# facebookresearch/gtn

Hardware: AMD Instinct MI355X
Metric: CTC forward+backward losses/sec (T=1000, C=256) (higher is better)
Workload: dtype f32; 1 GPU; BASELINE config C3: compose(ctc_target, emissions)+forwardScore CTC loss fwd+bwd, T=1000, C=256, U=100, batch=512 per GPU; global_batch=512, parallelism=dp1 (utterance sharding, all_gather of losses), rccl_ranks=0

## Files before the change

gtn_amd/_capi.py:

```python
import ctypes as C
import os

c_graph = C.c_void_p
c_graph_p = C.POINTER(C.c_void_p)
c_i32_p = C.POINTER(C.c_int)
c_i64_p = C.POINTER(C.c_int64)
c_u8_p = C.POINTER(C.c_uint8)
c_f32_p = C.POINTER(C.c_float)

GRAD_FN = C.CFUNCTYPE(C.c_int, C.c_void_p, c_graph_p, C.c_int, c_graph)
CTX_FREE = C.CFUNCTYPE(None, C.c_void_p)

OK, INVALID_ARGUMENT, LOGIC_ERROR, RUNTIME_ERROR, OUT_OF_RANGE, DEVICE_ERROR = range(6)

_SIGS = {
    "gtnx_set_device": [C.c_int],
    "gtnx_get_device": [c_i32_p],
    "gtnx_set_stream": [C.c_void_p],
    "gtnx_compose_mode": [C.c_int, C.POINTER(C.c_int)],
    "gtnx_synchronize": [],
    "gtnx_memory_stats": [C.POINTER(C.c_uint64), C.POINTER(C.c_uint64)],
    "gtnx_empty_cache": [],
    "gtnx_reclaim": [],
    "gtnx_graph_create": [C.c_int, c_graph_p],
# ... 55 lines not shown
    "gtnx_compose": [c_graph, c_graph, c_graph_p],
    "gtnx_intersect": [c_graph, c_graph, c_graph_p],
    "gtnx_forward_score": [c_graph, c_graph_p],
    "gtnx_viterbi_score": [c_graph, c_graph_p],
    "gtnx_viterbi_path": [c_graph, c_graph_p],
    "gtnx_negate_n": [c_graph_p, C.c_int, c_graph_p],
    "gtnx_add_n": [c_graph_p, C.c_int, c_graph_p, C.c_int, c_graph_p],
    "gtnx_subtract_n": [c_graph_p, C.c_int, c_graph_p, C.c_int, c_graph_p],
    "gtnx_compose_n": [c_graph_p, C.c_int, c_graph_p, C.c_int, c_graph_p],
    "gtnx_intersect_n": [c_graph_p, C.c_int, c_graph_p, C.c_int, c_graph_p],
    "gtnx_forward_score_n": [c_graph_p, C.c_int, c_graph_p],
    "gtnx_viterbi_score_n": [c_graph_p, C.c_int, c_graph_p],
    "gtnx_viterbi_path_n": [c_graph_p, C.c_int, c_graph_p],
    "gtnx_items_n": [c_graph_p, C.c_int, C.c_void_p],
    "gtnx_items_device_n": [c_graph_p, C.c_int, C.c_void_p],
    "gtnx_grads_device_n": [c_graph_p, C.c_int, C.c_void_p, C.c_void_p],
    "gtnx_grads_bind_device_n": [c_graph_p, C.c_int, C.c_void_p, C.c_void_p],
    "gtnx_clone": [c_graph, C.c_int, c_graph_p],
    "gtnx_concat": [c_graph_p, C.c_int, c_graph_p],
    "gtnx_closure": [c_graph, c_graph_p],
    "gtnx_union": [c_graph_p, C.c_int, c_graph_p],
    "gtnx_batch_from_graphs": [c_graph_p, C.c_int, c_graph_p],
    "gtnx_batch_ctc_targets": [C.c_void_p, C.c_void_p, C.c_int, C.c_int, C.c_int, c_graph_p],
    "gtnx_batch_asg_force_align": [C.c_void_p, C.c_void_p, C.c_int, c_graph, C.c_int, c_graph_p],
    "gtnx_batch_linear": [C.c_int, C.c_int, C.c_int, C.c_int, C.c_void_p, C.c_int, c_graph_p],
    "gtnx_batch_linear_rows": [C.c_int, C.c_int, C.c_int, C.c_void_p, C.c_int, C.c_void_p, C.c_int, c_graph_p],
    "gtnx_batch_destroy": [c_graph],
    "gtnx_batch_size": [c_graph, c_i32_p],
    "gtnx_batch_get": [c_graph, C.c_int, c_graph_p],
    "gtnx_batch_negate": [c_graph, c_graph_p],
    "gtnx_batch_add": [c_graph, c_graph, c_graph_p],
    "gtnx_batch_subtract": [c_graph, c_graph, c_graph_p],
    "gtnx_batch_subtract_into": [c_graph, c_graph, C.c_void_p, c_graph_p],
    "gtnx_batch_compose": [c_graph, c_graph, c_graph_p],
    "gtnx_batch_intersect": [c_graph, c_graph, c_graph_p],
    "gtnx_batch_forward_score": [c_graph, c_graph_p],
    "gtnx_batch_viterbi_score": [c_graph, c_graph_p],
    "gtnx_batch_viterbi_path": [c_graph, c_graph_p],
    "gtnx_batch_viterbi_align": [c_graph, C.c_void_p, C.c_void_p, C.c_int64, C.c_void_p, C.c_void_p],
    "gtnx_batch_align_stats": [c_i64_p, c_i64_p],
    "gtnx_batch_viterbi_decode": [c_graph, c_graph, C.c_void_p, C.c_void_p, C.c_int64, C.c_void_p, C.c_void_p,
                                  C.c_void_p],
    "gtnx_batch_decode_stats": [c_i64_p, c_i64_p],
    "gtnx_batch_full_connect_stats": [c_i64_p, c_i64_p],
    "gtnx_batch_linear_decode": [c_graph, C.c_void_p, C.c_int, C.c_void_p, C.c_int64, C.c_void_p, C.c_void_p,
                                 C.c_void_p, C.c_void_p],
# ... 85 lines not shown
```

gtn_amd/criteria/criteria_capi.cpp:

```cpp
#include <cstring>
#include <string>

#include <map>
#include <mutex>

#include "asg_criterion.h"
#include "ctc_criterion.h"
#include "edit_distance.h"

#define GTN_EXPORT extern "C" __attribute__((visibility("default")))

namespace {
thread_local std::string g_err;

template <class F>
int guarded(F&& body) {
  try {
    body();
    return 0;
  } catch (const std::exception& e) {
    g_err = e.what();
    return -1;
  }
}
// ... 78 lines not shown
                                    const void* weights, void* grad) {
  return guarded([&] {
    if (!weights || !grad) throw std::invalid_argument("gtn_ctc_score_grad_n: null weights or grad");
    gtn::criteria::ctcScoreBatch(emissions, B, T, C, blank, frames, tokens, lengths, N, L, max_length, nullptr, weights,
                                 grad);
  });
}

GTN_EXPORT int gtn_edit_distance_n(const void* hyp, const void* hyp_lengths, const void* ref, const void* ref_lengths,
                                   int B, int N, int L, int U, void* dist, void* ops) {
  return guarded([&] { gtn::criteria::editDistanceBatch(hyp, hyp_lengths, ref, ref_lengths, B, N, L, U, dist, ops); });
}

GTN_EXPORT int gtn_ctc_loss_target_grads_n(const void* emissions, const int* targets, const int* lengths, int B, int T,
                                           int C, int blank, void* loss, void* grad, void* target_grad,
                                           const int64_t* target_grad_offsets) {
  return guarded([&] {
    gtn::Batch ctcs;
    gtn::criteria::ctcLossBatch(emissions, targets, lengths, B, T, C, blank, loss, grad, true, nullptr, &ctcs);
    if (target_grad) ctcs.gradsToDevice(target_grad, target_grad_offsets);
  });
}

namespace {
void asg_loss_impl(const void* emissions, const int* targets, const int* lengths, int B, int T, int N, const void* trans_w,
                   const int* frames, void* loss, void* grad_em, void* grad_trans) {
  if (frames)
    for (int b = 0; b < B; ++b)
      if (frames[b] < 1 || frames[b] > T) throw std::invalid_argument("[gtn_asg_loss_frames_n] a frame count outside 1 .. T");
  std::lock_guard<std::mutex> lk(g_loss_transitions.mu);
  gtn::Graph& trans = transitions_for(g_loss_transitions, N, grad_trans != nullptr);
  trans.setCalcGrad(grad_trans != nullptr);
  trans.zeroGrad();
  trans.setWeightsDevice(trans_w);
  gtn::criteria::asgLossBatch(emissions, targets, lengths, B, T, N, trans, loss, grad_em, frames);
  if (grad_trans) {
    gtnx_graph_t h = trans.handle();
    int64_t off = 0;
    gtn::detail::check(gtnx_grads_device_n(&h, 1, grad_trans, &off));
  }
}
}

GTN_EXPORT int gtn_asg_loss_n(const void* emissions, const int* targets, const int* lengths, int B, int T, int N,
                              const void* trans_w, void* loss, void* grad_em, void* grad_trans) {
  return guarded([&] { asg_loss_impl(emissions, targets, lengths, B, T, N, trans_w, nullptr, loss, grad_em, grad_trans); });
// ... 31 lines not shown
```

gtn_amd/criteria/ctc_criterion.h:

```cpp
#pragma once

#include <chrono>
#include <cstdint>
#include <stdexcept>
#include <vector>

#include "gtn/gtn.h"

namespace gtn {
namespace criteria {

inline Graph ctcTargetGraph(const std::vector<int>& target, int blank = 0, bool calcGrad = true) {
  const int L = 2 * (int)target.size() + 1;
  std::vector<uint8_t> st(L, 0), ac(L, 0);
  std::vector<int> src, dst, lab;
  src.reserve(3 * L);
  dst.reserve(3 * L);
  lab.reserve(3 * L);
  for (int l = 0; l < L; l++) {
    const int idx = (l - 1) / 2;
    st[l] = l == 0;
    ac[l] = l == L - 1 || l + 2 == L;
    const int label = l % 2 ? target[idx] : blank;
    src.push_back(l), dst.push_back(l), lab.push_back(label);
// ... 10 lines not shown
struct CtcStepTimes {
  double build = 0, linear = 0, intersect = 0, forward = 0, backward = 0;
};

inline void ctcLossBatch(
    const void* emissions,
    const int* labels,
    const int* lengths,
    int B,
    int T,
    int C,
    int blank,
    void* lossDev,
    void* gradDev,
    bool targetGrad = true,
    CtcStepTimes* times = nullptr,
    Batch* targetsOut = nullptr,
    const int* frames = nullptr) {
  auto now = [] { return std::chrono::steady_clock::now(); };
  auto ms = [](auto a, auto b) { return std::chrono::duration<double, std::milli>(b - a).count(); };
  if (frames)
    for (int b = 0; b < B; ++b)
      if (frames[b] < 1 || frames[b] > T) throw std::invalid_argument("[ctcLossBatch] a frame count outside 1 .. T");
  auto t0 = now();
  Batch ctcs = Batch::ctcTargets(labels, lengths, B, blank, targetGrad);
  auto t1 = now();
  Batch ems = Batch::linear(B, T, C, emissions, gradDev != nullptr, true, frames);
  std::vector<int64_t> off(B);
  for (int b = 0; b < B; ++b) off[b] = (int64_t)b * T * C;
  if (gradDev) ems.bindGrads(gradDev, off.data());
  auto t2 = now();
  Batch comp = batched::intersect(ctcs, ems);
  auto t3 = now();
  Batch score = batched::forwardScore(comp);
  Batch norm = batched::forwardScore(ems);
  Batch losses = batched::subtract(norm, score, lossDev);
  auto t4 = now();
  if (gradDev) batched::backward(losses);
  auto t5 = now();
  if (times) *times = {ms(t0, t1), ms(t1, t2), ms(t2, t3), ms(t3, t4), ms(t4, t5)};
  losses.itemsToDevice(lossDev);
  if (gradDev) ems.gradsToDevice(gradDev, off.data());
  if (targetsOut) *targetsOut = std::move(ctcs);
}

inline void ctcLossBatch(
// ... 128 lines not shown
```

gtn_amd/csrc/band.hip:

```cpp
#include <hip/hip_runtime.h>

#include <algorithm>
#include <cstdlib>
#include <stdexcept>
#include <type_traits>

#include "kernels.h"

#ifdef GTNX_BAND_TIMING
__device__ long long g_band_timing[256];
#endif

namespace gtnx {
namespace {

constexpr float NEGF = -1.0e30f;
constexpr float DEADF = -1.0e29f;
constexpr float LOG2E = 1.44269504088896340736f;
constexpr double LN2 = 0.693147180559945309417;
constexpr int BW = 256;
constexpr int WG = 512;
constexpr int WGB = 768;
constexpr int NBE = 5;
constexpr int NBG = 7;
// ... 302 lines not shown

__device__ __forceinline__ float wave_max_of(const float* v, int n) {
  float mx = v[0];
  for (int j = 1; j < n; ++j) mx = fmaxf(mx, v[j]);
  return wave_max(mx);
}

template <int NPL, bool UNIT, int K, bool VEC>
__global__ __launch_bounds__(WG) void band_forward_kernel(const BandPair* __restrict__ pairs, int NSmax) {
#define GTNX_BAND_PAIR pairs[blockIdx.x]
#include "band_forward_body.inc"
#undef GTNX_BAND_PAIR
}
template <int NPL, bool UNIT, int K, bool VEC>
__global__ __launch_bounds__(WG) void band_forward_one_kernel(BandPair one, int NSmax) {
#define GTNX_BAND_PAIR one
#include "band_forward_body.inc"
#undef GTNX_BAND_PAIR
}

__device__ __forceinline__ BandPair band_patched(BandPair P, const BandPatch& pt) {
  if (pt.on) {
    const int b = P.bidx;
    P.delta = pt.delta + b;
    P.delta_norm = pt.delta_norm ? pt.delta_norm + b : nullptr;
    P.rowlse = pt.rowlse ? pt.rowlse + int64_t(b) * pt.M : nullptr;
    P.norm = nullptr;
    P.em_copy = nullptr;
    P.grad_em = pt.grad_em ? pt.grad_em + int64_t(b) * pt.A : nullptr;
    P.grad_fixed = pt.grad_fixed ? pt.grad_fixed + P.goff : nullptr;
  }
  return P;
}
template <int NPL, bool UNIT, bool GRADG, int K, bool VEC, bool BIG>
__global__ __launch_bounds__(WGB, BIG ? 3 : 6) void band_backward_kernel(const BandPair* __restrict__ pairs, int NSmax, BandPatch patch) {
#define GTNX_BAND_PAIR band_patched(pairs[blockIdx.x], patch)
#include "band_backward_body.inc"
#undef GTNX_BAND_PAIR
}
template <int NPL, bool UNIT, bool GRADG, int K, bool VEC, bool BIG>
__global__ __launch_bounds__(WGB, BIG ? 3 : 6) void band_backward_one_kernel(BandPair one, int NSmax) {
#define GTNX_BAND_PAIR one
#include "band_backward_body.inc"
#undef GTNX_BAND_PAIR
}


__global__ __launch_bounds__(512) void ctc_targets_kernel(const CtcTargetArgs* __restrict__ args, int blank) {
  const CtcTargetArgs a = args[blockIdx.x];
  __shared__ __attribute__((aligned(16))) int tl[256 + 4];
  __shared__ __attribute__((aligned(16))) int tk[256 + 4];
  const int N = a.N, U = (N - 1) >> 1, m = threadIdx.x;
  if (m < 260) {
    const int v = m < U ? a.labels[m] : 0x7fffffff;
    tl[m] = v;
    tk[m] = (m > 0 && m < U && v != a.labels[m - 1]) ? 1 : 0;
  }
  __syncthreads();
  if (m >= N) return;
  const bool odd = (m & 1) != 0;
  const int my = odd ? tl[(m - 1) >> 1] : blank;
  const int skip = odd ? tk[(m - 1) >> 1] : 0;
  const int mi = (m - 1) >> 1;
  const int before = odd ? mi : (m >> 1);
  int rank = 0, skips = 0;
  for (int o = 0; o < U; o += 4) {
    const gtnx_i4 l4 = *reinterpret_cast<const gtnx_i4*>(tl + o), k4 = *reinterpret_cast<const gtnx_i4*>(tk + o);
    const int lo[4] = {l4.x, l4.y, l4.z, l4.w}, ko[4] = {k4.x, k4.y, k4.z, k4.w};
#pragma unroll
    for (int k = 0; k < 4; ++k) {
      const bool front = o + k < before;
      rank += (lo[k] < my || (lo[k] == my && front)) ? 1 : 0;
      skips += front ? ko[k] : 0;
    }
  }
  rank += blank < my ? U + 1 : (blank == my ? (m + 1) >> 1 : 0);
  const int base = (m > 0 ? 2 * m - 1 : 0) + skips;
  GTNX_G BandNode* nd = const_cast<GTNX_G BandNode*>(a.nodes);
  nd[m].lab = my;
  nd[m].aid[0] = base;
  nd[m].aid[1] = m > 0 ? base + 1 : -1;
  nd[m].aid[2] = skip ? base + 2 : -1;
  a.nflags[m] = uint8_t((m == 0 ? NF_START : 0) | (m + 2 >= N ? NF_ACCEPT : 0));
  a.snode[rank] = m;
  a.slab[rank] = my;
  if (m == N - 1 && a.n_arcs) a.n_arcs[0] = base + 1 + (m > 0 ? 1 : 0) + skip;
}

__global__ __launch_bounds__(512) void band_viterbi_kernel(const BandDecode* __restrict__ pairs) {
  const BandDecode P = pairs[blockIdx.x];
  const int T = P.T, C = P.C, N = P.N, NS = P.NS;
  extern __shared__ float lds[];
  const float NINF = -__builtin_inff();
  float* a0 = lds;
  float* a1 = lds + 516;
  float* stage = lds + 1032;
  const int m = threadIdx.x;
  const GTNX_G gtnx_i4* nodes = reinterpret_cast<const GTNX_G gtnx_i4*>(P.nodes);
  int lab = 0;
  float wi[3] = {NINF, NINF, NINF};
  bool accept = false, start = false;
  if (m < N) {
    const gtnx_i4 q = nodes[m];
    lab = q.x >= 0 ? q.x : 0;
    const int a[3] = {q.y, q.z, q.w};
#pragma unroll
    for (int k = 0; k < 3; ++k)
      if (a[k] >= 0) wi[k] = P.w ? P.w[a[k]] : 0.0f;
    const uint8_t f = P.nflags[m];
// ... 539 lines not shown
    else if (max_nodes <= 128) launch_viterbi_wave<2>(d_pairs, n, ranked, st);
    else if (max_nodes <= 256) launch_viterbi_wave<4>(d_pairs, n, ranked, st);
    else launch_viterbi_wave<8>(d_pairs, n, ranked, st);
    return;
  }
  if (ranked) return;
  static std::atomic<uint64_t> done{0};
  if (gtnx_first_on_device first{done}) big_lds(band_viterbi_kernel);
  hipLaunchKernelGGL(band_viterbi_kernel, dim3(n), dim3(512), 4 * size_t(1032 + stage_floats) + 64, st, d_pairs);
}

void launch_asg_fal_targets(const AsgFalArgs* d_args, int n, int n_labels, hipStream_t st) {
  if (n > 0) hipLaunchKernelGGL(asg_fal_targets_kernel, dim3(n), dim3(512), 0, st, d_args, n_labels);
}
void launch_asg_fal_scatter(const float* g, const int* maps, const int64_t* tab, int n_seq, int64_t longest, float* trans_grad,
                            hipStream_t st) {
  if (n_seq > 0 && longest > 0)
    hipLaunchKernelGGL(asg_fal_scatter_kernel, dim3(unsigned(std::min<int64_t>((longest + 255) / 256, 64)), unsigned(n_seq)),
                       dim3(256), 0, st, g, maps, tab, trans_grad);
}
void launch_ctc_targets(const CtcTargetArgs* d_args, int n, int blank, hipStream_t st) {
  if (n > 0) hipLaunchKernelGGL(ctc_targets_kernel, dim3(n), dim3(512), 0, st, d_args, blank);
}

}
```

gtn_amd/csrc/band_backward_body.inc:

```
  constexpr int RNk = K >= 4 ? 4 : K;
  constexpr int NP = K / RNk;
  const BandPair P = GTNX_BAND_PAIR;
  const int T = P.T, C = P.C, NS = P.NS;
  extern __shared__ float lds[];
  const BandLds L = band_lds(C, K, NSmax, true);
  float* ering = lds + L.o_ering;
  float* aring = lds + L.o_aring;
  float* oring = lds + L.o_oring;
  int* snode = reinterpret_cast<int*>(lds + L.o_snode);
  const BandMisc M = band_misc<K>(lds, L);
  float* lser = M.lsep;
  const int CS = L.CS;
  const int wv = __builtin_amdgcn_readfirstlane(threadIdx.x >> 6);
  const bool sweeper = wv < 4;
  const int l = threadIdx.x & 63;
  const int nblocks = (T + K - 1) / K;
  const int nticks = nblocks + 5;
  const GTNX_G double* ao = P.aoff;
  const double z2 = uniform(ao[0]);
  const bool dead = !(z2 > double(DEADF));
  const float ds = uniform(P.delta[0]);
  const bool want_em = P.grad_em != nullptr;
  GTNX_TM_INIT(128);
  constexpr bool SPLIT = !BIG && K >= 2 && GTNX_BWD_SPLIT;
  const float dn_k = P.delta_norm ? uniform(P.delta_norm[0]) : 0.0f;
  float* const rnorm_k = lser + NBG * K;
  auto rows_of_k = [&](int c) { return c < nblocks ? min(K, T - c * K) : 0; };
  auto ring_start = [](int c, int M) { return ((c % M) + M) % M; };
  static_assert((NBGE & (NBGE - 1)) == 0, "the emission ring's position is a mask");
  auto ge_of = [](int c) { return int(unsigned(c) & unsigned(NBGE - 1)); };
  auto ring_step = [](int& v, int M) { v = v + 1 == M ? 0 : v + 1; };
  struct RowSumRegs {
    float in[NPL];
    gtnx_f4 hot[NPL];
  };
  auto rowsum_init = [&](RowSumRegs& R) {
#pragma unroll
    for (int q = 0; q < NPL; ++q) {
      const int mb = 256 * q + 4 * l;
      R.in[q] = mb < NSmax ? 1.0f : 0.0f;
      float hm[4];
#pragma unroll
      for (int k = 0; k < 4; ++k) {
        const int m = mb + k;
        int lab = -1;
        if (m < P.N) lab = P.nodes[m].lab;
        settle(lab);
        hm[k] = (P.hot >= 0 && lab == P.hot) ? 1.0f : 0.0f;
// ... 680 lines not shown
```

gtn_amd/csrc/band_forward_body.inc:

```
#ifndef GTNX_FWD_SHIFT_ROWS
#define GTNX_FWD_SHIFT_ROWS 4
#endif
  constexpr int RNk = K >= GTNX_FWD_SHIFT_ROWS ? GTNX_FWD_SHIFT_ROWS : (K >= 4 ? 4 : K);
  constexpr int NP = K / RNk;
  constexpr int D = 8 / K > GTNX_FWD_DEPTH ? 8 / K : GTNX_FWD_DEPTH;
  const BandPair P = GTNX_BAND_PAIR;
  const int T = P.T, C = P.C, NS = P.NS;
  extern __shared__ float lds[];
  const BandLds L = band_lds(C, K, NSmax, false);
  float* ering = lds + L.o_ering;
  const BandMisc M = band_misc<K>(lds, L);
  const int CS = L.CS;
  const int wv = __builtin_amdgcn_readfirstlane(threadIdx.x >> 6);
  const bool sweeper = wv < 4;
  const int l = threadIdx.x & 63;
  const int nblocks = (T + K - 1) / K;
  const int nticks = nblocks + 3;
  GTNX_TM_INIT(0);

  if (sweeper) {
    __builtin_amdgcn_s_setprio(1);
    const int w = wv;
    const int m0 = threadIdx.x * NPL;
    NodeRegs<NPL> g;
// ... 309 lines not shown
        }
      }
    };
    if (em_copy) {
      if (GTNX_FWD_COPY_ROTATE) run_copy();
      else run(std::true_type{});
    } else {
      run(std::false_type{});
    }
    if (hid < 16) M.red[hid] = normacc;
  }
  GTNX_TM_DUMP();
  lds_barrier();
  if (threadIdx.x == 0) {
    double Mx = double(NEGF);
    for (int k = 0; k < 4; ++k)
      if (M.fin[2 * k] > DEADF) Mx = fmax(Mx, M.find[k] + double(M.fin[2 * k]));
    const bool dead = !(Mx > double(DEADF));
    float S = 0.0f;
    for (int k = 0; k < 4; ++k)
      if (M.fin[2 * k] > DEADF) S += M.fin[2 * k + 1] * ex2(float(M.find[k] + double(M.fin[2 * k]) - Mx));
    const double z2 = dead ? double(NEGF) : Mx + double(lg2(S));
    P.aoff[0] = z2;
    P.score[0] = dead ? -__builtin_inff() : float(z2 * LN2);
    if (P.norm) {
      double n2 = 0.0;
      for (int k = 0; k < 16; ++k) n2 += M.red[k];
      P.norm[0] = n2 < double(DEADF) ? -__builtin_inff() : float(n2 * LN2);
    }
  }
```

gtn_amd/csrc/batch.h:

```cpp
#pragma once

#include <memory>
#include <vector>

#include "ops.h"

namespace gtnx {

struct Batch;
using BatchP = std::shared_ptr<Batch>;

struct BatchOp {
  uint64_t seq = 0;
  std::vector<BatchP> inputs;
  virtual void backward(Batch& out) = 0;
  virtual ~BatchOp() {}
};

struct Batch {
  enum Kind { GRAPHS, CTC_TARGETS, LINEAR, PRODUCT, SCALAR };
  Kind kind = GRAPHS;
  int n = 0;
  bool calc_grad = false;

// ... 32 lines not shown
  DevMemP pad_mem;
  int rows_of(int b) const { return rows.empty() ? M : rows[size_t(b)]; }
  BatchP fixed, chain;
  bool chain_first = false, intersect = false;
  bool wide = false;
  bool full = false;
  DevMemP v_mem;
  float* v_dev = nullptr;

  std::shared_ptr<BatchOp> op;
  bool tape_cleared = false;
  DevMemP g_mem;
  float* g_dev = nullptr;
  std::vector<int64_t> g_off;
  DevMemP dest_mem;
  float* dest = nullptr;

  int64_t elem_size(int b) const;
  ~Batch();
};

BatchP batch_from_graphs(std::vector<Graph> gs);
BatchP batch_ctc_targets(const int* labels, const int* lengths, int n, int blank, bool calc_grad);
BatchP batch_asg_force_align(const int* labels, const int* lengths, int n, Graph& transitions, int n_labels);
BatchP batch_linear(int n, int M, int C, bool calc_grad, const void* dev, bool borrow, const int* rows = nullptr);
BatchP batch_compose(const BatchP& a, const BatchP& b, bool intersect);
BatchP batch_shortest_distance(const BatchP& x, bool tropical);
void batch_full_connect_stats(int64_t* fast, int64_t* fallback);
BatchP batch_viterbi_path(const BatchP& x);
void batch_viterbi_align(const BatchP& x, const int* frames, int* labels_dev, int64_t row_stride, int* tokens_dev,
                         float* scores_dev);
void batch_align_stats(int64_t* fast, int64_t* fallback);
void batch_viterbi_decode(const BatchP& ems, Graph& transitions, const int* frames, int* labels_dev, int64_t row_stride,
                          float* scores_dev, int* collapsed_dev, int* lengths_dev);
void batch_decode_stats(int64_t* fast, int64_t* fallback);
void batch_linear_decode(const BatchP& ems, const int* frames, int blank, int* labels_dev, int64_t row_stride,
                         float* scores_dev, int* collapsed_dev, int* starts_dev, int* lengths_dev);
void batch_linear_decode_stats(int64_t* fast, int64_t* fallback);
void batch_ctc_beam_decode(const BatchP& ems, const int* frames, int blank, int beam, int topn, int nbest,
                           int* tokens_dev, int64_t row_stride, int* lengths_dev, float* scores_dev);
struct CtcBeamLm {
  const float* table_dev;
  float weight, bonus;
  float* am_scores_dev;
};
void batch_ctc_beam_decode(const BatchP& ems, const int* frames, int blank, int beam, int topn, int nbest,
// ... 27 lines not shown
```

gtn_amd/csrc/capi.cpp:

```cpp
#include <atomic>
#include <chrono>
#include <condition_variable>
#include <cstdlib>
#include <cstring>
#include <mutex>
#include <string>
#include <vector>

#include "batch.h"
#include "ops.h"
#include "ops_internal.h"
#include "region.h"

#define GTNX_API extern "C" __attribute__((visibility("default")))

using namespace gtnx;

namespace {
thread_local std::string g_err;

gtnx_status_t fail(gtnx_status_t s, const std::string& m) {
  g_err = m;
  return s;
}
// ... 722 lines not shown
    auto v = vec(g, n);
    *out = H(op_rational(RAT_UNION, v, 0));
  });
}

GTNX_API gtnx_status_t gtnx_remove(gtnx_graph_t g, int ilabel, int olabel, gtnx_graph_t* out) {
  return guard([&] { *out = H(op_remove(G(g), ilabel, olabel)); });
}

namespace {
inline BatchP& BH(gtnx_batch_t h) {
  if (!h) throw_invalid("null batch handle");
  return *reinterpret_cast<BatchP*>(h);
}
inline gtnx_batch_t HB(BatchP b) { return reinterpret_cast<gtnx_batch_t>(new BatchP(std::move(b))); }
}
GTNX_API gtnx_status_t gtnx_batch_from_graphs(const gtnx_graph_t* g, int n, gtnx_batch_t* out) {
  return guard([&] { *out = HB(batch_from_graphs(vec(g, n, true))); });
}
GTNX_API gtnx_status_t gtnx_batch_ctc_targets(const int* labels, const int* lengths, int n, int blank, int cg,
                                              gtnx_batch_t* out) {
  return guard([&] { *out = HB(batch_ctc_targets(labels, lengths, n, blank, cg != 0)); });
}
GTNX_API gtnx_status_t gtnx_batch_asg_force_align(const int* labels, const int* lengths, int n, gtnx_graph_t transitions,
                                                  int n_labels, gtnx_batch_t* out) {
  return guard([&] { *out = HB(batch_asg_force_align(labels, lengths, n, G(transitions), n_labels)); });
}
GTNX_API gtnx_status_t gtnx_batch_linear(int n, int M, int N, int cg, const void* dev, int borrow, gtnx_batch_t* out) {
  return guard([&] { *out = HB(batch_linear(n, M, N, cg != 0, dev, borrow != 0)); });
}
GTNX_API gtnx_status_t gtnx_batch_linear_rows(int n, int M, int N, const int* rows, int cg, const void* dev, int borrow,
                                             gtnx_batch_t* out) {
  return guard([&] { *out = HB(batch_linear(n, M, N, cg != 0, dev, borrow != 0, rows)); });
}
GTNX_API gtnx_status_t gtnx_batch_destroy(gtnx_batch_t b) {
  return guard([&] {
    auto* p = reinterpret_cast<BatchP*>(b);
    if (!p) return;
    if (Runtime::initialized())
      Runtime::get().defer_delete(p, [](void* q) { delete static_cast<BatchP*>(q); },
                                  (*p && (*p)->materialised) ? size_t((*p)->n > 0 ? (*p)->n : 1) : 1);
    else
      delete p;
  });
}
GTNX_API gtnx_status_t gtnx_batch_size(gtnx_batch_t b, int* out) {
// ... 235 lines not shown
```

gtn_amd/csrc/kernels.h:

```cpp
#pragma once

#include <hip/hip_runtime.h>

#include <cstdint>

#include <atomic>
#include <cstdint>
struct gtnx_first_on_device {
  std::atomic<uint64_t>& done;
  uint64_t bit;
  bool first;
  explicit gtnx_first_on_device(std::atomic<uint64_t>& d) : done(d) {
    int dev = 0;
    (void)hipGetDevice(&dev);
    bit = uint64_t(1) << (dev & 63);
    first = !(done.load(std::memory_order_acquire) & bit);
  }
  gtnx_first_on_device(const gtnx_first_on_device&) = delete;
  ~gtnx_first_on_device() {
    if (first) done.fetch_or(bit, std::memory_order_acq_rel);
  }
  explicit operator bool() const { return first; }
};

// ... 332 lines not shown
struct BandPair {
  const GTNX_G BandNode* nodes;
  const GTNX_G uint8_t* nflags;
  const GTNX_G int* snode;
  const GTNX_G int* slab;
  const GTNX_G float* w;
  const GTNX_G float* em;
  GTNX_G float* em_copy;
  GTNX_G float* alpha;
  GTNX_G double* aoff;
  GTNX_G float* score;
  GTNX_G float* norm;
  GTNX_G float* rowlse;
  const GTNX_G float* delta;
  const GTNX_G float* delta_norm;
  GTNX_G float* grad_em;
  GTNX_G float* grad_fixed;
  int N, T, C, NS;
  int hot;
  int lgrn;
  int n_lab;
  int bidx;
  int64_t goff;
};
struct BandPatch {
  int on;
  int M;
  const GTNX_G float* delta;
  const GTNX_G float* delta_norm;
  GTNX_G float* rowlse;
  GTNX_G float* grad_em;
  GTNX_G float* grad_fixed;
  int64_t A;
};
struct BandDecode {
  const GTNX_G BandNode* nodes;
  const GTNX_G uint8_t* nflags;
  const GTNX_G float* w;
  const GTNX_G float* em;
  GTNX_G uint8_t* bp;
  GTNX_G int* pnode;
  GTNX_G int* path_arc;
  GTNX_G int* path_lab;
  GTNX_G float* path_w;
  GTNX_G int* path_len;
  GTNX_G float* score;
  GTNX_G int* tie;
  const GTNX_G int* rank_in;
  const GTNX_G int* rank_acc;
  int N, T, C, NS;
  int stage_floats, pad;
};
void launch_band_viterbi(const BandDecode* d_pairs, int n, int stage_floats, int max_nodes, int max_labels, int vec,
                         hipStream_t st, int ranked = 0);
bool band_viterbi_wave_ok(int max_nodes, int max_labels, int vec);
struct AlignArgs {
// ... 61 lines not shown
  GTNX_G int* stamp;
  GTNX_G int* queue;
  GTNX_G int* arc_cnt;
  const GTNX_G int* arc_off;
  RationalOut out;
};
void launch_remove_keep(const DGraph& g, int ilabel, int olabel, int* keep, hipStream_t st);
void launch_remove_roots(const int* keep, const int* new_id, int N, int* roots, hipStream_t st);
void launch_remove_walk(const RemoveArgs& a, bool emit, hipStream_t st);
size_t scan_temp_bytes(int n);
void launch_exclusive_scan(const int* in, int* out, int n, void* temp, size_t temp_bytes, hipStream_t st);
void launch_rational_load(const void* rows, const float* w, const uint8_t* flags, const RationalOut& out, void* temp,
                          hipStream_t st);
struct CtcTargetArgs {
  const GTNX_G int* labels;
  GTNX_G BandNode* nodes;
  GTNX_G uint8_t* nflags;
  GTNX_G int* snode;
  GTNX_G int* slab;
  GTNX_G int* n_arcs;
  int N, pad;
};
void launch_ctc_targets(const CtcTargetArgs* d_args, int n, int blank, hipStream_t st);
struct AsgFalArgs {
  const GTNX_G int* labels;
  const GTNX_G float* trans_w;
  GTNX_G BandNode* nodes;
  GTNX_G uint8_t* nflags;
  GTNX_G int* snode;
  GTNX_G int* slab;
  GTNX_G float* w;
  GTNX_G int* arc_map;
  int U, pad;
};
void launch_asg_fal_targets(const AsgFalArgs* d_args, int n, int n_labels, hipStream_t st);
void launch_asg_fal_scatter(const float* g, const int* maps, const int64_t* tab , int n_seq, int64_t longest,
                            float* trans_grad, hipStream_t st);
int band_max_nodes();
int band_max_labels();
int band_min_labels();
int band_npl(int max_nodes);
int band_row_stride(int N, int npl);
int band_forward_lgrn(int C);
bool band_one_ok(int npl, int C, int max_NS, bool vec, bool backward);
void launch_band_forward(const BandPair* d_pairs, int n, int npl, int C, int max_NS, bool unit, bool vec, hipStream_t st,
                         const BandPair* one = nullptr);
// ... 158 lines not shown
```

include/gtn/batch.h:

```cpp
#pragma once
#include <cstdint>
#include <utility>
#include <vector>

#include "gtn/functions.h"

namespace gtn {

class Batch {
 public:
  Batch() = default;
  explicit Batch(const std::vector<Graph>& graphs) {
    auto h = detail::handles(graphs);
    detail::check(gtnx_batch_from_graphs(h.data(), static_cast<int>(h.size()), &h_));
  }
  Batch(const Batch&) = delete;
  Batch& operator=(const Batch&) = delete;
  Batch(Batch&& o) noexcept : h_(o.h_) { o.h_ = nullptr; }
  Batch& operator=(Batch&& o) noexcept {
    if (this != &o) {
      reset();
      h_ = o.h_;
      o.h_ = nullptr;
    }
// ... 34 lines not shown
  }

  int size() const {
    int n = 0;
    if (h_) detail::check(gtnx_batch_size(h_, &n));
    return n;
  }
  Graph operator[](int i) const {
    gtnx_graph_t g;
    detail::check(gtnx_batch_get(h_, i, &g));
    return Graph::fromHandle(g);
  }
  std::vector<float> items() const {
    std::vector<float> v(static_cast<size_t>(size()));
    if (!v.empty()) detail::check(gtnx_batch_items(h_, v.data()));
    return v;
  }
  void itemsToDevice(void* deviceOut) const { detail::check(gtnx_batch_items_device(h_, deviceOut)); }
  void bindGrads(void* deviceOut, const int64_t* offsets) { detail::check(gtnx_batch_grads_bind_device(h_, deviceOut, offsets)); }
  void gradsToDevice(void* deviceOut, const int64_t* offsets) const {
    detail::check(gtnx_batch_grads_device(h_, deviceOut, offsets));
  }
  gtnx_batch_t handle() const { return h_; }
  static Batch fromHandle(gtnx_batch_t h) {
    Batch b;
    b.h_ = h;
    return b;
  }

 private:
  void reset() {
    if (h_) gtnx_batch_destroy(h_);
    h_ = nullptr;
  }
  gtnx_batch_t h_ = nullptr;
};

namespace detail {
template <class F>
Batch batchUnary(F f, const Batch& a) {
  gtnx_batch_t out;
  check(f(a.handle(), &out));
  return Batch::fromHandle(out);
}
template <class F>
Batch batchBinary(F f, const Batch& a, const Batch& b) {
// ... 44 lines not shown
                          float* amScoresDevice = nullptr, int blank = 0, int beamSize = 16, int cutoffTopN = 16,
                          int nbest = 1, const int* frames = nullptr) {
  detail::check(gtnx_batch_ctc_beam_decode_lm(ems.handle(), frames, blank, beamSize, cutoffTopN, nbest, lmDevice,
                                              lmWeight, insertionBonus, tokensDevice, rowStride, lengthsDevice,
                                              scoresDevice, amScoresDevice));
}
inline void editDistance(const int* hypDevice, int64_t hypStride, const int* hypLengthsDevice, const int* refDevice,
                         int64_t refStride, const int* refLengthsDevice, int B, int N, int L, int U, int* distDevice,
                         int* opsDevice = nullptr) {
  detail::check(gtnx_batch_edit_distance(hypDevice, hypStride, hypLengthsDevice, refDevice, refStride, refLengthsDevice,
                                         B, N, L, U, distDevice, opsDevice));
}
inline void ctcScore(const Batch& ems, const int* tokensDevice, int64_t rowStride, const int* lengthsDevice, int N, int L,
                     int maxLength, float* scoresDevice, int blank = 0, const int* frames = nullptr) {
  detail::check(gtnx_batch_ctc_score(ems.handle(), frames, blank, tokensDevice, rowStride, lengthsDevice, N, L, maxLength,
                                     scoresDevice));
}
inline void ctcScoreGrad(const Batch& ems, const int* tokensDevice, int64_t rowStride, const int* lengthsDevice, int N,
                         int L, int maxLength, const float* weightsDevice, float* gradDevice, int blank = 0,
                         const int* frames = nullptr) {
  detail::check(gtnx_batch_ctc_score_grad(ems.handle(), frames, blank, tokensDevice, rowStride, lengthsDevice, N, L,
                                          maxLength, weightsDevice, gradDevice));
}
inline void backward(const Batch& a, bool retainGraph = false) { detail::check(gtnx_batch_backward(a.handle(), retainGraph)); }
}

}
```

include/gtn_amd.h:

```cpp
#ifndef GTN_AMD_H
#define GTN_AMD_H

#include <stddef.h>
#include <stdint.h>

#ifdef __cplusplus
extern "C" {
#endif

typedef int gtnx_status_t;
#define GTNX_OK 0
#define GTNX_INVALID_ARGUMENT 1
#define GTNX_LOGIC_ERROR 2
#define GTNX_RUNTIME_ERROR 3
#define GTNX_OUT_OF_RANGE 4
#define GTNX_DEVICE_ERROR 5

typedef struct gtnx_graph_s* gtnx_graph_t;

#define GTNX_EPSILON (-1)

const char* gtnx_last_error(void);
const char* gtnx_version(void);
const char* gtnx_backend(void);
// ... 87 lines not shown
gtnx_status_t gtnx_negate_n(const gtnx_graph_t* g, int n, gtnx_graph_t* out);
gtnx_status_t gtnx_add_n(const gtnx_graph_t* a, int na, const gtnx_graph_t* b, int nb, gtnx_graph_t* out);
gtnx_status_t gtnx_subtract_n(const gtnx_graph_t* a, int na, const gtnx_graph_t* b, int nb, gtnx_graph_t* out);
gtnx_status_t gtnx_compose_n(const gtnx_graph_t* a, int na, const gtnx_graph_t* b, int nb, gtnx_graph_t* out);
gtnx_status_t gtnx_intersect_n(const gtnx_graph_t* a, int na, const gtnx_graph_t* b, int nb, gtnx_graph_t* out);
gtnx_status_t gtnx_forward_score_n(const gtnx_graph_t* g, int n, gtnx_graph_t* out);
gtnx_status_t gtnx_viterbi_score_n(const gtnx_graph_t* g, int n, gtnx_graph_t* out);
gtnx_status_t gtnx_viterbi_path_n(const gtnx_graph_t* g, int n, gtnx_graph_t* out);
gtnx_status_t gtnx_items_n(const gtnx_graph_t* g, int n, float* out);
gtnx_status_t gtnx_items_device_n(const gtnx_graph_t* g, int n, void* device_out);
gtnx_status_t gtnx_grads_device_n(const gtnx_graph_t* g, int n, void* device_out, const int64_t* offsets);
gtnx_status_t gtnx_grads_bind_device_n(const gtnx_graph_t* g, int n, void* device_out, const int64_t* offsets);

gtnx_status_t gtnx_clone(gtnx_graph_t g, int projection , gtnx_graph_t* out);
gtnx_status_t gtnx_concat(const gtnx_graph_t* g, int n, gtnx_graph_t* out);
gtnx_status_t gtnx_closure(gtnx_graph_t g, gtnx_graph_t* out);
gtnx_status_t gtnx_union(const gtnx_graph_t* g, int n, gtnx_graph_t* out);
gtnx_status_t gtnx_remove(gtnx_graph_t g, int ilabel, int olabel, gtnx_graph_t* out);

typedef struct gtnx_batch_s* gtnx_batch_t;
gtnx_status_t gtnx_batch_from_graphs(const gtnx_graph_t* g, int n, gtnx_batch_t* out);
gtnx_status_t gtnx_batch_ctc_targets(const int* labels, const int* lengths, int n, int blank, int calc_grad,
                                     gtnx_batch_t* out);
gtnx_status_t gtnx_batch_asg_force_align(const int* labels, const int* lengths, int n, gtnx_graph_t transitions,
                                         int n_labels, gtnx_batch_t* out);
gtnx_status_t gtnx_batch_linear(int n, int M, int N, int calc_grad, const void* device_weights, int borrow,
                                gtnx_batch_t* out);
gtnx_status_t gtnx_batch_linear_rows(int n, int M, int N, const int* rows, int calc_grad, const void* device_weights,
                                     int borrow, gtnx_batch_t* out);
gtnx_status_t gtnx_batch_destroy(gtnx_batch_t b);
gtnx_status_t gtnx_batch_size(gtnx_batch_t b, int* out);
gtnx_status_t gtnx_batch_get(gtnx_batch_t b, int i, gtnx_graph_t* out);
gtnx_status_t gtnx_batch_negate(gtnx_batch_t a, gtnx_batch_t* out);
gtnx_status_t gtnx_batch_add(gtnx_batch_t a, gtnx_batch_t b, gtnx_batch_t* out);
gtnx_status_t gtnx_batch_subtract(gtnx_batch_t a, gtnx_batch_t b, gtnx_batch_t* out);
gtnx_status_t gtnx_batch_subtract_into(gtnx_batch_t a, gtnx_batch_t b, void* items_device, gtnx_batch_t* out);
gtnx_status_t gtnx_batch_compose(gtnx_batch_t a, gtnx_batch_t b, gtnx_batch_t* out);
gtnx_status_t gtnx_batch_intersect(gtnx_batch_t a, gtnx_batch_t b, gtnx_batch_t* out);
gtnx_status_t gtnx_batch_forward_score(gtnx_batch_t a, gtnx_batch_t* out);
gtnx_status_t gtnx_batch_viterbi_score(gtnx_batch_t a, gtnx_batch_t* out);
gtnx_status_t gtnx_batch_viterbi_path(gtnx_batch_t a, gtnx_batch_t* out);
gtnx_status_t gtnx_batch_viterbi_align(gtnx_batch_t a, const int* frames, void* labels_device, int64_t row_stride,
                                       void* tokens_device, void* scores_device);
gtnx_status_t gtnx_batch_align_stats(int64_t* fast, int64_t* fallback);
gtnx_status_t gtnx_batch_viterbi_decode(gtnx_batch_t ems, gtnx_graph_t transitions, const int* frames,
                                        void* labels_device, int64_t row_stride, void* scores_device,
// ... 65 lines not shown
```

Baseline: 1.013 million losses/s.

## Add fused CTC loss step that builds targets, band table and runs forward/backward

Adds a fused path for batched CTC loss with gradients. A single head kernel builds the CTC target records, the per-utterance band pair table and the arena layout on device from pinned labels. The forward band kernel then writes the loss directly, and the backward kernel uses constant deltas instead of device-side delta buffers. This removes the separate target-batch construction, compose, subtract and backward-seed steps, along with their host work and kernel launches. In exchange it adds a new code path with several fallback conditions to the generic route.

```diff
diff --git a/gtn_amd/_capi.py b/gtn_amd/_capi.py
--- a/gtn_amd/_capi.py
+++ b/gtn_amd/_capi.py
@@ -101,6 +101,8 @@
     "gtnx_union": [c_graph_p, C.c_int, c_graph_p],
     "gtnx_batch_from_graphs": [c_graph_p, C.c_int, c_graph_p],
     "gtnx_batch_ctc_targets": [C.c_void_p, C.c_void_p, C.c_int, C.c_int, C.c_int, c_graph_p],
+    "gtnx_batch_ctc_loss_step": [C.c_void_p, C.c_void_p, C.c_void_p, C.c_int, C.c_int, C.c_int, C.c_int, C.c_void_p,
+                                 C.c_void_p, C.c_int, C.POINTER(C.c_double), c_graph_p, c_i32_p],
     "gtnx_batch_asg_force_align": [C.c_void_p, C.c_void_p, C.c_int, c_graph, C.c_int, c_graph_p],
     "gtnx_batch_linear": [C.c_int, C.c_int, C.c_int, C.c_int, C.c_void_p, C.c_int, c_graph_p],
     "gtnx_batch_linear_rows": [C.c_int, C.c_int, C.c_int, C.c_void_p, C.c_int, C.c_void_p, C.c_int, c_graph_p],
diff --git a/gtn_amd/criteria/criteria_capi.cpp b/gtn_amd/criteria/criteria_capi.cpp
--- a/gtn_amd/criteria/criteria_capi.cpp
+++ b/gtn_amd/criteria/criteria_capi.cpp
@@ -124,6 +124,17 @@
   });
 }
 
+GTN_EXPORT int gtn_ctc_loss_targets_n(const void* emissions, const int* targets, const int* lengths, int B, int T, int C,
+                                      int blank, const int* frames, void* loss, void* grad, int target_grad,
+                                      void** targets_out) {
+  return guarded([&] {
+    gtn::Batch ctcs;
+    gtn::criteria::ctcLossBatch(emissions, targets, lengths, B, T, C, blank, loss, grad, target_grad != 0, nullptr,
+                                targets_out ? &ctcs : nullptr, frames);
+    if (targets_out) *targets_out = ctcs.release();
+  });
+}
+
 namespace {
 void asg_loss_impl(const void* emissions, const int* targets, const int* lengths, int B, int T, int N, const void* trans_w,
                    const int* frames, void* loss, void* grad_em, void* grad_trans) {
diff --git a/gtn_amd/criteria/ctc_criterion.h b/gtn_amd/criteria/ctc_criterion.h
--- a/gtn_amd/criteria/ctc_criterion.h
+++ b/gtn_amd/criteria/ctc_criterion.h
@@ -56,6 +56,13 @@
   if (frames)
     for (int b = 0; b < B; ++b)
       if (frames[b] < 1 || frames[b] > T) throw std::invalid_argument("[ctcLossBatch] a frame count outside 1 .. T");
+  if (gradDev && !frames && B > 1) {
+    double hostMs[3] = {0, 0, 0};
+    if (batched::ctcLossStep(emissions, labels, lengths, B, T, C, blank, lossDev, gradDev, targetGrad, hostMs, targetsOut)) {
+      if (times) *times = {hostMs[0], 0, 0, hostMs[1], hostMs[2]};
+      return;
+    }
+  }
   auto t0 = now();
   Batch ctcs = Batch::ctcTargets(labels, lengths, B, blank, targetGrad);
   auto t1 = now();
diff --git a/gtn_amd/csrc/band.hip b/gtn_amd/csrc/band.hip
--- a/gtn_amd/csrc/band.hip
+++ b/gtn_amd/csrc/band.hip
@@ -348,9 +348,9 @@
 __device__ __forceinline__ BandPair band_patched(BandPair P, const BandPatch& pt) {
   if (pt.on) {
     const int b = P.bidx;
-    P.delta = pt.delta + b;
-    P.delta_norm = pt.delta_norm ? pt.delta_norm + b : nullptr;
+    P.delta = pt.delta ? pt.delta + b : nullptr;
     P.rowlse = pt.rowlse ? pt.rowlse + int64_t(b) * pt.M : nullptr;
+    P.delta_norm = pt.delta_norm ? pt.delta_norm + b : P.rowlse;
     P.norm = nullptr;
     P.em_copy = nullptr;
     P.grad_em = pt.grad_em ? pt.grad_em + int64_t(b) * pt.A : nullptr;
@@ -358,30 +358,45 @@
   }
   return P;
 }
+__device__ __forceinline__ float band_delta(const BandPair& P, const BandPatch& pt) {
+  return (pt.on && !pt.delta) ? pt.delta_const : uniform(P.delta[0]);
+}
+__device__ __forceinline__ float band_delta_norm(const BandPair& P, const BandPatch& pt) {
+  return (pt.on && !pt.delta_norm) ? pt.delta_norm_const : uniform(P.delta_norm[0]);
+}
 template <int NPL, bool UNIT, bool GRADG, int K, bool VEC, bool BIG>
 __global__ __launch_bounds__(WGB, BIG ? 3 : 6) void band_backward_kernel(const BandPair* __restrict__ pairs, int NSmax, BandPatch patch) {
 #define GTNX_BAND_PAIR band_patched(pairs[blockIdx.x], patch)
+#define GTNX_BAND_DELTA(P) band_delta(P, patch)
+#define GTNX_BAND_DELTA_NORM(P) band_delta_norm(P, patch)
 #include "band_backward_body.inc"
+#undef GTNX_BAND_DELTA_NORM
+#undef GTNX_BAND_DELTA
 #undef GTNX_BAND_PAIR
 }
 template <int NPL, bool UNIT, bool GRADG, int K, bool VEC, bool BIG>
 __global__ __launch_bounds__(WGB, BIG ? 3 : 6) void band_backward_one_kernel(BandPair one, int NSmax) {
 #define GTNX_BAND_PAIR one
+#define GTNX_BAND_DELTA(P) uniform((P).delta[0])
+#define GTNX_BAND_DELTA_NORM(P) uniform((P).delta_norm[0])
 #include "band_backward_body.inc"
+#undef GTNX_BAND_DELTA_NORM
+#undef GTNX_BAND_DELTA
 #undef GTNX_BAND_PAIR
 }
 
 
-__global__ __launch_bounds__(512) void ctc_targets_kernel(const CtcTargetArgs* __restrict__ args, int blank) {
-  const CtcTargetArgs a = args[blockIdx.x];
+__device__ __forceinline__ void ctc_target_records(const CtcTargetArgs& a, int label, bool store_labels, int blank) {
   __shared__ __attribute__((aligned(16))) int tl[256 + 4];
   __shared__ __attribute__((aligned(16))) int tk[256 + 4];
   const int N = a.N, U = (N - 1) >> 1, m = threadIdx.x;
   if (m < 260) {
-    const int v = m < U ? a.labels[m] : 0x7fffffff;
+    const int v = m < U ? label : 0x7fffffff;
     tl[m] = v;
-    tk[m] = (m > 0 && m < U && v != a.labels[m - 1]) ? 1 : 0;
-  }
+    if (store_labels && m < U) const_cast<GTNX_G int*>(a.labels)[m] = v;
+  }
+  __syncthreads();
+  if (m < 260) tk[m] = (m > 0 && m < U && tl[m] != tl[m - 1]) ? 1 : 0;
   __syncthreads();
   if (m >= N) return;
   const bool odd = (m & 1) != 0;
@@ -411,6 +426,57 @@
   a.snode[rank] = m;
   a.slab[rank] = my;
   if (m == N - 1 && a.n_arcs) a.n_arcs[0] = base + 1 + (m > 0 ? 1 : 0) + skip;
+}
+__global__ __launch_bounds__(512) void ctc_targets_kernel(const CtcTargetArgs* __restrict__ args, int blank) {
+  const CtcTargetArgs a = args[blockIdx.x];
+  const int m = threadIdx.x;
+  ctc_target_records(a, 2 * m + 1 < a.N ? a.labels[m] : 0, false, blank);
+}
+__global__ __launch_bounds__(512) void ctc_step_head_kernel(CtcStepHead h) {
+  const int b = blockIdx.x;
+  const int label = int(threadIdx.x) < h.lab_stride ? h.labels[int64_t(b) * h.lab_stride + threadIdx.x] : 0;
+  const CtcStepUtt u = h.utt[b];
+  const int N = u.N;
+  CtcTargetArgs a;
+  GTNX_G char* rec = h.rec_mem + u.rec_off;
+  a.labels = reinterpret_cast<const GTNX_G int*>(h.rec_mem) + u.lab_off;
+  a.nodes = reinterpret_cast<GTNX_G BandNode*>(rec);
+  rec += (int64_t(sizeof(BandNode)) * N + 63) / 64 * 64;
+  a.nflags = reinterpret_cast<GTNX_G uint8_t*>(rec);
+  rec += (int64_t(N) + 63) / 64 * 64;
+  a.snode = reinterpret_cast<GTNX_G int*>(rec);
+  rec += (4 * int64_t(N) + 63) / 64 * 64;
+  a.slab = reinterpret_cast<GTNX_G int*>(rec);
+  rec += (4 * int64_t(N) + 63) / 64 * 64;
+  a.n_arcs = reinterpret_cast<GTNX_G int*>(rec);
+  a.N = N;
+  a.pad = 0;
+  if (threadIdx.x == 0) {
+    h.args[b] = a;
+    BandPair p{};
+    p.nodes = a.nodes;
+    p.nflags = a.nflags;
+    p.snode = a.snode;
+    p.slab = a.slab;
+    p.em = h.em + int64_t(b) * h.em_stride;
+    p.alpha = reinterpret_cast<GTNX_G float*>(h.arena + u.alpha_off);
+    p.aoff = reinterpret_cast<GTNX_G double*>(h.arena + u.shift_off);
+    p.score = reinterpret_cast<GTNX_G float*>(h.arena) + b;
+    p.norm = reinterpret_cast<GTNX_G float*>(h.arena + h.o_norm) + b;
+    p.rowlse = reinterpret_cast<GTNX_G float*>(h.arena + h.o_lse) + int64_t(b) * h.T;
+    p.N = N;
+    p.T = h.T;
+    p.C = h.C;
+    p.NS = (N + 3) / 4 * 4;
+    p.hot = ((N - 1) / 2 + 1 >= 8) ? h.blank : -1;
+    p.lgrn = h.lgrn;
+    p.n_lab = N;
+    p.bidx = b;
+    p.goff = u.goff;
+    p.loss = h.loss + b;
+    h.table[b] = p;
+  }
+  ctc_target_records(a, label, true, h.blank);
 }
 
 __global__ __launch_bounds__(512) void band_viterbi_kernel(const BandDecode* __restrict__ pairs) {
@@ -996,5 +1062,8 @@
 void launch_ctc_targets(const CtcTargetArgs* d_args, int n, int blank, hipStream_t st) {
   if (n > 0) hipLaunchKernelGGL(ctc_targets_kernel, dim3(n), dim3(512), 0, st, d_args, blank);
 }
-
-}
+void launch_ctc_step_head(const CtcStepHead& h, int n, hipStream_t st) {
+  if (n > 0) hipLaunchKernelGGL(ctc_step_head_kernel, dim3(n), dim3(512), 0, st, h);
+}
+
+}
diff --git a/gtn_amd/csrc/band_backward_body.inc b/gtn_amd/csrc/band_backward_body.inc
--- a/gtn_amd/csrc/band_backward_body.inc
+++ b/gtn_amd/csrc/band_backward_body.inc
@@ -19,11 +19,11 @@
   const GTNX_G double* ao = P.aoff;
   const double z2 = uniform(ao[0]);
   const bool dead = !(z2 > double(DEADF));
-  const float ds = uniform(P.delta[0]);
+  const float ds = GTNX_BAND_DELTA(P);
   const bool want_em = P.grad_em != nullptr;
   GTNX_TM_INIT(128);
   constexpr bool SPLIT = !BIG && K >= 2 && GTNX_BWD_SPLIT;
-  const float dn_k = P.delta_norm ? uniform(P.delta_norm[0]) : 0.0f;
+  const float dn_k = P.delta_norm ? GTNX_BAND_DELTA_NORM(P) : 0.0f;
   float* const rnorm_k = lser + NBG * K;
   auto rows_of_k = [&](int c) { return c < nblocks ? min(K, T - c * K) : 0; };
   auto ring_start = [](int c, int M) { return ((c % M) + M) % M; };
diff --git a/gtn_amd/csrc/band_forward_body.inc b/gtn_amd/csrc/band_forward_body.inc
--- a/gtn_amd/csrc/band_forward_body.inc
+++ b/gtn_amd/csrc/band_forward_body.inc
@@ -355,10 +355,14 @@
       if (M.fin[2 * k] > DEADF) S += M.fin[2 * k + 1] * ex2(float(M.find[k] + double(M.fin[2 * k]) - Mx));
     const double z2 = dead ? double(NEGF) : Mx + double(lg2(S));
     P.aoff[0] = z2;
-    P.score[0] = dead ? -__builtin_inff() : float(z2 * LN2);
+    const float score = dead ? -__builtin_inff() : float(z2 * LN2);
+    P.score[0] = score;
     if (P.norm) {
       double n2 = 0.0;
       for (int k = 0; k < 16; ++k) n2 += M.red[k];
-      P.norm[0] = n2 < double(DEADF) ? -__builtin_inff() : float(n2 * LN2);
+      const float norm = n2 < double(DEADF) ? -__builtin_inff() : float(n2 * LN2);
+      P.norm[0] = norm;
+      GTNX_G float* const loss = (GTNX_BAND_PAIR).loss;
+      if (loss) loss[0] = norm - score;
     }
   }
diff --git a/gtn_amd/csrc/batch.h b/gtn_amd/csrc/batch.h
--- a/gtn_amd/csrc/batch.h
+++ b/gtn_amd/csrc/batch.h
@@ -78,6 +78,8 @@
 
 BatchP batch_from_graphs(std::vector<Graph> gs);
 BatchP batch_ctc_targets(const int* labels, const int* lengths, int n, int blank, bool calc_grad);
+bool batch_ctc_loss_step(const void* em_dev, const int* labels, const int* lengths, int n, int T, int C, int blank,
+                         void* loss_dev, void* grad_dev, bool target_grad, double* host_ms, BatchP* targets_out);
 BatchP batch_asg_force_align(const int* labels, const int* lengths, int n, Graph& transitions, int n_labels);
 BatchP batch_linear(int n, int M, int C, bool calc_grad, const void* dev, bool borrow, const int* rows = nullptr);
 BatchP batch_compose(const BatchP& a, const BatchP& b, bool intersect);
diff --git a/gtn_amd/csrc/capi.cpp b/gtn_amd/csrc/capi.cpp
--- a/gtn_amd/csrc/capi.cpp
+++ b/gtn_amd/csrc/capi.cpp
@@ -768,6 +768,20 @@
                                               gtnx_batch_t* out) {
   return guard([&] { *out = HB(batch_ctc_targets(labels, lengths, n, blank, cg != 0)); });
 }
+GTNX_API gtnx_status_t gtnx_batch_ctc_loss_step(const void* emissions_device, const int* labels, const int* lengths, int n,
+                                                int T, int C, int blank, void* loss_device, void* grad_device,
+                                                int target_grad, double* host_ms, gtnx_batch_t* targets_out, int* taken) {
+  return guard([&] {
+    if (!taken) throw_invalid("[gtnx_batch_ctc_loss_step] null `taken`");
+    if (targets_out) *targets_out = nullptr;
+    BatchP targets;
+    *taken = batch_ctc_loss_step(emissions_device, labels, lengths, n, T, C, blank, loss_device, grad_device,
+                                 target_grad != 0, host_ms, targets_out ? &targets : nullptr)
+                 ? 1
+                 : 0;
+    if (*taken && targets_out) *targets_out = HB(std::move(targets));
+  });
+}
 GTNX_API gtnx_status_t gtnx_batch_asg_force_align(const int* labels, const int* lengths, int n, gtnx_graph_t transitions,
                                                   int n_labels, gtnx_batch_t* out) {
   return guard([&] { *out = HB(batch_asg_force_align(labels, lengths, n, G(transitions), n_labels)); });
diff --git a/gtn_amd/csrc/ctc_step.cpp b/gtn_amd/csrc/ctc_step.cpp
--- /dev/null
+++ b/gtn_amd/csrc/ctc_step.cpp
@@ -0,0 +1,167 @@
+#include "batch.h"
+
+#include <algorithm>
+#include <chrono>
+#include <cstdlib>
+#include <cstring>
+
+namespace gtnx {
+
+bool batch_ctc_loss_step(const void* em_dev, const int* labels, const int* lengths, int n, int T, int C, int blank,
+                         void* loss_dev, void* grad_dev, bool target_grad, double* host_ms, BatchP* targets_out) {
+  GTNX_HOST_T("batch.ctc_loss_step");
+  if (!em_dev || !lengths || !loss_dev) throw_invalid("[gtnx_batch_ctc_loss_step] null emissions, lengths or loss");
+  for (const char* sw : {"GTNX_H2D_KERNEL_BYTES", "GTNX_NO_BAND_PATCH", "GTNX_LAZY_COMPOSE"})
+    if (std::getenv(sw)) return false;
+  if (const char* e = std::getenv("GTNX_CTC_STEP_FUSED"))
+    if (std::strcmp(e, "0") == 0) return false;
+  if (!grad_dev || n <= 1 || T < 1 || T > (1 << 20) || C < band_min_labels() || C > band_max_labels() || blank < 0 ||
+      blank >= C)
+    return false;
+  int64_t total = 0;
+  int max_nodes = 0, min_nodes = 1 << 30;
+  for (int i = 0; i < n; ++i) {
+    if (lengths[i] < 0) throw_invalid("[gtnx_batch_ctc_loss_step] negative length");
+    total += lengths[i];
+    if (lengths[i] > band_max_nodes()) return false;
+    max_nodes = std::max(max_nodes, 2 * lengths[i] + 1);
+    min_nodes = std::min(min_nodes, 2 * lengths[i] + 1);
+  }
+  if (total > 0 && !labels) throw_invalid("[gtnx_batch_ctc_loss_step] null labels");
+  if (max_nodes > band_max_nodes() || band_npl(max_nodes) != band_npl(min_nodes)) return false;
+  int max_label = blank;
+  for (int64_t i = 0; i < total; ++i) {
+    if (labels[i] < 0) return false;
+    max_label = std::max(max_label, labels[i]);
+  }
+  if (max_label >= C) return false;
+
+  auto now = [] { return std::chrono::steady_clock::now(); };
+  auto ms = [](auto a, auto b) { return std::chrono::duration<double, std::milli>(b - a).count(); };
+  const auto t0 = now();
+  Runtime& rt = Runtime::get();
+  BatchP b = std::make_shared<Batch>();
+  b->kind = Batch::CTC_TARGETS;
+  b->n = n;
+  b->calc_grad = target_grad;
+  b->blank = blank;
+  b->lab_off.resize(size_t(n) + 1);
+  b->lab_off[0] = 0;
+  for (int i = 0; i < n; ++i) b->lab_off[size_t(i) + 1] = b->lab_off[size_t(i)] + lengths[i];
+  b->max_nodes = max_nodes;
+  b->max_label = max_label;
+  if (total > 0) b->labels.assign(labels, labels + total);
+  const size_t lab_bytes = align_up(sizeof(int) * size_t(total ? total : 1), 256);
+  const size_t arg_bytes = align_up(sizeof(CtcTargetArgs) * size_t(n), 256);
+  size_t rec_bytes = lab_bytes + arg_bytes;
+  b->rec_off.resize(size_t(n));
+  for (int i = 0; i < n; ++i) {
+    const size_t N = size_t(2 * lengths[i] + 1);
+    b->rec_off[size_t(i)] = rec_bytes;
+    rec_bytes += align_up(sizeof(BandNode) * N, 64) + align_up(N, 64) + 2 * align_up(4 * N, 64) + 64;
+  }
+  b->rec_mem = rt.alloc(rec_bytes);
+  size_t bytes = align_up(4 * size_t(n), 256);
+  const size_t o_norm = bytes;
+  bytes = align_up(bytes + 4 * size_t(n), 256);
+  const size_t o_lse = bytes;
+  bytes = align_up(bytes + 4 * size_t(n) * size_t(T), 256);
+  const int lab_stride = std::max(4, (max_nodes - 1) / 2);
+  const size_t pin_lab_bytes = align_up(sizeof(int) * size_t(n) * size_t(lab_stride), 256);
+  const size_t utt_bytes = sizeof(CtcStepUtt) * size_t(n);
+  PinnedMemP pin = rt.alloc_pinned(pin_lab_bytes + utt_bytes);
+  for (int i = 0; i < n; ++i)
+    if (lengths[i] > 0)
+      std::memcpy(pin->as<int>() + size_t(i) * size_t(lab_stride), labels + b->lab_off[size_t(i)],
+                  sizeof(int) * size_t(lengths[i]));
+  CtcStepUtt* utt = pin->as<CtcStepUtt>(pin_lab_bytes);
+  int max_ns = 0;
+  int64_t goff_run = 0;
+  double fwd_bytes = 0, bwd_bytes = 0;
+  std::vector<int64_t> g_off(size_t(n) + 1);
+  for (int i = 0; i < n; ++i) {
+    const int N = 2 * lengths[i] + 1;
+    const int ns = band_row_stride(N, band_npl(N));
+    CtcStepUtt& u = utt[size_t(i)];
+    u.lab_off = b->lab_off[size_t(i)];
+    u.rec_off = int64_t(b->rec_off[size_t(i)]);
+    u.shift_off = int64_t(bytes);
+    bytes = align_up(bytes + 8 * (4 * size_t(T) + 16), 256);
+    u.alpha_off = int64_t(bytes);
+    bytes = align_up(bytes + 4 * size_t(T + 1) * size_t(ns), 256);
+    u.goff = goff_run;
+    u.N = N;
+    u.pad = 0;
+    g_off[size_t(i)] = goff_run;
+    goff_run += b->elem_size(i);
+    max_ns = std::max(max_ns, ns);
+    fwd_bytes += 4.0 * T * C + 4.0 * double(T + 1) * ns;
+    bwd_bytes += 4.0 * T * C * 2 + 4.0 * double(T + 1) * ns + (target_grad ? 4.0 * double(b->elem_size(i)) : 0.0);
+  }
+  g_off[size_t(n)] = goff_run;
+  DevMemP arena = rt.alloc(bytes);
+  DevMemP table = rt.alloc(sizeof(BandPair) * size_t(n));
+  const size_t A = size_t(T) * size_t(C);
+  CtcStepHead h{};
+  h.labels = pin->as<int>();
+  h.utt = utt;
+  h.rec_mem = b->rec_mem->as<char>();
+  h.args = b->rec_mem->as<CtcTargetArgs>(lab_bytes);
+  h.table = table->as<BandPair>();
+  h.em = static_cast<const float*>(em_dev);
+  h.em_stride = int64_t(A);
+  h.arena = arena->as<char>();
+  h.o_norm = int64_t(o_norm);
+  h.o_lse = int64_t(o_lse);
+  h.loss = static_cast<float*>(loss_dev);
+  h.C = C;
+  h.T = T;
+  h.blank = blank;
+  h.lgrn = band_forward_lgrn(C);
+  h.lab_stride = lab_stride;
+  {
+    GTNX_PROF("ctc_step_head", double(pin_lab_bytes + utt_bytes));
+    launch_ctc_step_head(h, n, rt.stream());
+  }
+  pin.reset();
+  const auto t1 = now();
+  const int npl = band_npl(max_nodes);
+  const bool vec = C % 4 == 0 && (reinterpret_cast<uintptr_t>(em_dev) & 15) == 0;
+  {
+    GTNX_PROF("band_forward_score", fwd_bytes);
+    launch_band_forward(table->as<BandPair>(), n, npl, C, max_ns, true, vec, rt.stream());
+  }
+  const auto t2 = now();
+  if (target_grad) {
+    b->g_off = std::move(g_off);
+    const size_t gbytes = sizeof(float) * size_t(goff_run);
+    b->g_mem = rt.alloc(gbytes ? gbytes : 4);
+    b->g_dev = b->g_mem->as<float>();
+  }
+  BandPatch pt{};
+  pt.on = 1;
+  pt.M = T;
+  pt.delta = nullptr;
+  pt.delta_norm = nullptr;
+  pt.delta_const = -1.0f;
+  pt.delta_norm_const = 1.0f;
+  pt.rowlse = arena->as<float>(o_lse);
+  pt.grad_em = static_cast<float*>(grad_dev);
+  pt.grad_fixed = b->g_dev;
+  pt.A = int64_t(A);
+  {
+    GTNX_PROF("band_forward_score_grad", bwd_bytes);
+    launch_band_backward(table->as<BandPair>(), n, npl, C, max_ns, true, target_grad, vec, rt.stream(),
+                         nullptr, &pt);
+  }
+  const auto t3 = now();
+  if (host_ms) {
+    host_ms[0] = ms(t0, t1);
+    host_ms[1] = ms(t1, t2);
+    host_ms[2] = ms(t2, t3);
+  }
+  if (targets_out) *targets_out = std::move(b);
+  return true;
+}
+
+}
diff --git a/gtn_amd/csrc/kernels.h b/gtn_amd/csrc/kernels.h
--- a/gtn_amd/csrc/kernels.h
+++ b/gtn_amd/csrc/kernels.h
@@ -378,6 +378,7 @@
   int n_lab;
   int bidx;
   int64_t goff;
+  GTNX_G float* loss;
 };
 struct BandPatch {
   int on;
@@ -388,6 +389,7 @@
   GTNX_G float* grad_em;
   GTNX_G float* grad_fixed;
   int64_t A;
+  float delta_const, delta_norm_const;
 };
 struct BandDecode {
   const GTNX_G BandNode* nodes;
@@ -495,6 +497,29 @@
   int N, pad;
 };
 void launch_ctc_targets(const CtcTargetArgs* d_args, int n, int blank, hipStream_t st);
+struct CtcStepUtt {
+  int64_t lab_off;
+  int64_t rec_off;
+  int64_t shift_off;
+  int64_t alpha_off;
+  int64_t goff;
+  int N, pad;
+};
+struct CtcStepHead {
+  const GTNX_G int* labels;
+  const GTNX_G CtcStepUtt* utt;
+  GTNX_G char* rec_mem;
+  CtcTargetArgs* args;
+  BandPair* table;
+  const GTNX_G float* em;
+  int64_t em_stride;
+  GTNX_G char* arena;
+  int64_t o_norm, o_lse;
+  GTNX_G float* loss;
+  int C, T, blank, lgrn;
+  int lab_stride, pad;
+};
+void launch_ctc_step_head(const CtcStepHead& h, int n, hipStream_t st);
 struct AsgFalArgs {
   const GTNX_G int* labels;
   const GTNX_G float* trans_w;
diff --git a/include/gtn/batch.h b/include/gtn/batch.h
--- a/include/gtn/batch.h
+++ b/include/gtn/batch.h
@@ -80,6 +80,11 @@
     detail::check(gtnx_batch_grads_device(h_, deviceOut, offsets));
   }
   gtnx_batch_t handle() const { return h_; }
+  gtnx_batch_t release() {
+    gtnx_batch_t h = h_;
+    h_ = nullptr;
+    return h;
+  }
   static Batch fromHandle(gtnx_batch_t h) {
     Batch b;
     b.h_ = h;
@@ -170,6 +175,16 @@
   detail::check(gtnx_batch_ctc_score_grad(ems.handle(), frames, blank, tokensDevice, rowStride, lengthsDevice, N, L,
                                           maxLength, weightsDevice, gradDevice));
 }
+inline bool ctcLossStep(const void* emissionsDevice, const int* labels, const int* lengths, int n, int T, int C, int blank,
+                        void* lossDevice, void* gradDevice, bool targetGrad = true, double* hostMs = nullptr,
+                        Batch* targetsOut = nullptr) {
+  gtnx_batch_t targets = nullptr;
+  int taken = 0;
+  detail::check(gtnx_batch_ctc_loss_step(emissionsDevice, labels, lengths, n, T, C, blank, lossDevice, gradDevice,
+                                         targetGrad, hostMs, targetsOut ? &targets : nullptr, &taken));
+  if (taken && targetsOut) *targetsOut = Batch::fromHandle(targets);
+  return taken != 0;
+}
 inline void backward(const Batch& a, bool retainGraph = false) { detail::check(gtnx_batch_backward(a.handle(), retainGraph)); }
 }
 
diff --git a/include/gtn_amd.h b/include/gtn_amd.h
--- a/include/gtn_amd.h
+++ b/include/gtn_amd.h
@@ -133,6 +133,9 @@
 gtnx_status_t gtnx_batch_from_graphs(const gtnx_graph_t* g, int n, gtnx_batch_t* out);
 gtnx_status_t gtnx_batch_ctc_targets(const int* labels, const int* lengths, int n, int blank, int calc_grad,
                                      gtnx_batch_t* out);
+gtnx_status_t gtnx_batch_ctc_loss_step(const void* emissions_device, const int* labels, const int* lengths, int n, int T,
+                                       int C, int blank, void* loss_device, void* grad_device, int target_grad,
+                                       double* host_ms, gtnx_batch_t* targets_out, int* taken);
 gtnx_status_t gtnx_batch_asg_force_align(const int* labels, const int* lengths, int n, gtnx_graph_t transitions,
                                          int n_labels, gtnx_batch_t* out);
 gtnx_status_t gtnx_batch_linear(int n, int M, int N, int calc_grad, const void* device_weights, int borrow,
```

Result: faster. 1.042 million losses/s (median of 6 runs) (+2.8%).
